# davidfang00/opticalflowdiffusion

Measured on NVIDIA B200. Metric: flows/sec DDIM-50 @436x1024, higher is better.
Workload: dtype bf16

## Files before the change

opticalflowdiffusion_b200/csrc/fd_attention.cu:

```cuda
#include <stdlib.h>

#include "fd_mma.cuh"

using namespace fdmma;

namespace {


constexpr int kLaTile = 64;
constexpr int kLaRowBytes = 2 * kHidden * 2 + 16;
constexpr int kLaTileBytes = kLaTile * kLaRowBytes;
constexpr int kLaSmemBytes = 2 * kLaTileBytes;
constexpr int kLaPartial = 2 * kHidden + kHeads * kD * kD;

__global__ void __launch_bounds__(256, 3) linattn_partial_kernel(const __nv_bfloat16* __restrict__ kv, int row_stride,
                                                              float* __restrict__ partial, int HW, int chunk_px) {
  extern __shared__ __align__(16) uint8_t la_smem[];
  const int n = blockIdx.y, chunk = blockIdx.x;
  const int p_begin = chunk * chunk_px;
  const int p_end = min(HW, p_begin + chunk_px);
  const int t = threadIdx.x, warp = t >> 5, lane = t & 31;
  const int g = lane >> 2, tq = lane & 3;
  const int head = warp & 3, mhalf = warp >> 2;
  const __nv_bfloat16* base = kv + (long)n * HW * row_stride;
// ... 27 lines not shown
      issue_tile(p0 + kLaTile, buf ^ 1);
      cp_async_wait<1>();
    } else {
      cp_async_wait<0>();
    }
    __syncthreads();
    const uint32_t tb = smem0 + buf * kLaTileBytes;
    const int nvalid = p_end - p0;
    uint32_t ka[kLaTile / 16][4];
#pragma unroll
    for (int ks = 0; ks < kLaTile / 16; ++ks)
      ldmatrix_x4_trans(ka[ks], tb + (ks * 16 + (mi >> 1) * 8 + r) * kLaRowBytes + (head * kD + mhalf * 16 + (mi & 1) * 8) * 2);
    float t0 = -INFINITY, t1 = -INFINITY;
#pragma unroll
    for (int ks = 0; ks < kLaTile / 16; ++ks) {
#pragma unroll
      for (int rg = 0; rg < 4; ++rg) {
        const float2 f = fd_unpack_bf16(ka[ks][rg]);
        const int px = ks * 16 + 2 * tq + (rg >> 1) * 8;
        const float a = px < nvalid ? f.x : -INFINITY, b = px + 1 < nvalid ? f.y : -INFINITY;
        if (rg & 1) t1 = fmaxf(t1, fmaxf(a, b)); else t0 = fmaxf(t0, fmaxf(a, b));
      }
    }
    t0 = fmaxf(t0, __shfl_xor_sync(0xffffffffu, t0, 1)); t0 = fmaxf(t0, __shfl_xor_sync(0xffffffffu, t0, 2));
    t1 = fmaxf(t1, __shfl_xor_sync(0xffffffffu, t1, 1)); t1 = fmaxf(t1, __shfl_xor_sync(0xffffffffu, t1, 2));
    const float mn0 = fmaxf(m0, t0), mn1 = fmaxf(m1, t1);
    const float f0 = (m0 == -INFINITY) ? 0.f : __expf(m0 - mn0), f1 = (m1 == -INFINITY) ? 0.f : __expf(m1 - mn1);
    m0 = mn0;
    m1 = mn1;
#pragma unroll
    for (int nt = 0; nt < 4; ++nt) {
      acc[nt][0] *= f0; acc[nt][1] *= f0; acc[nt][2] *= f1; acc[nt][3] *= f1;
    }
    float e0 = 0.f, e1 = 0.f;
#pragma unroll
    for (int ks = 0; ks < kLaTile / 16; ++ks) {
#pragma unroll
      for (int rg = 0; rg < 4; ++rg) {
        const float2 f = fd_unpack_bf16(ka[ks][rg]);
        const int px = ks * 16 + 2 * tq + (rg >> 1) * 8;
        const float mm = (rg & 1) ? mn1 : mn0;
        const float a = px < nvalid ? __expf(f.x - mm) : 0.f, b = px + 1 < nvalid ? __expf(f.y - mm) : 0.f;
        const uint32_t pk = fd_pack_bf16(a, b);
        ka[ks][rg] = pk;
        const float2 rq = fd_unpack_bf16(pk);
        if (rg & 1) e1 += rq.x + rq.y; else e0 += rq.x + rq.y;
      }
    }
    s0 = s0 * f0 + e0;
    s1 = s1 * f1 + e1;
#pragma unroll
    for (int ks = 0; ks < kLaTile / 16; ++ks) {
      uint32_t b01[4], b23[4];
      const uint32_t vb = tb + (ks * 16 + (mi & 1) * 8 + r) * kLaRowBytes + (kHidden + head * kD + (mi >> 1) * 8) * 2;
      ldmatrix_x4_trans(b01, vb);
      ldmatrix_x4_trans(b23, vb + 16 * 2);
      mma_bf16(acc[0], ka[ks], b01[0], b01[1]);
      mma_bf16(acc[1], ka[ks], b01[2], b01[3]);
      mma_bf16(acc[2], ka[ks], b23[0], b23[1]);
      mma_bf16(acc[3], ka[ks], b23[2], b23[3]);
    }
    __syncthreads();
  }
  s0 += __shfl_xor_sync(0xffffffffu, s0, 1); s0 += __shfl_xor_sync(0xffffffffu, s0, 2);
  s1 += __shfl_xor_sync(0xffffffffu, s1, 1); s1 += __shfl_xor_sync(0xffffffffu, s1, 2);
  float* out = partial + ((long)n * gridDim.x + chunk) * kLaPartial;
  if (tq == 0) {
    const int d0 = head * kD + mhalf * 16 + g;
    out[d0] = m0;
    out[d0 + 8] = m1;
    out[kHidden + d0] = s0;
    out[kHidden + d0 + 8] = s1;
  }
  float* c = out + 2 * kHidden + (head * kD + mhalf * 16) * kD;
#pragma unroll
  for (int nt = 0; nt < 4; ++nt) {
    c[g * kD + nt * 8 + 2 * tq] = acc[nt][0];
    c[g * kD + nt * 8 + 2 * tq + 1] = acc[nt][1];
    c[(g + 8) * kD + nt * 8 + 2 * tq] = acc[nt][2];
    c[(g + 8) * kD + nt * 8 + 2 * tq + 1] = acc[nt][3];
  }
}

__global__ void __launch_bounds__(1024) linattn_combine_kernel(const float* __restrict__ partial,
                                                               __nv_bfloat16* __restrict__ ctx_t, int nchunks,
                                                               float inv_hw) {
  const int n = blockIdx.x / kHeads, head = blockIdx.x % kHeads;
  const int d = threadIdx.x >> 5, e = threadIdx.x & 31;
  const float* base = partial + (long)n * nchunks * kLaPartial;
  float M = -INFINITY;
  for (int c = 0; c < nchunks; ++c) M = fmaxf(M, base[(long)c * kLaPartial + head * kD + d]);
  float S = 0.f, acc = 0.f;
  for (int c = 0; c < nchunks; ++c) {
    const float* pc = base + (long)c * kLaPartial;
    const float mc = pc[head * kD + d];
    const float f = (mc == -INFINITY) ? 0.f : __expf(mc - M);
    S += pc[kHidden + head * kD + d] * f;
    acc += pc[2 * kHidden + (head * kD + d) * kD + e] * f;
  }
  ctx_t[((long)n * kHeads + head) * kD * kD + e * kD + d] = __float2bfloat16(acc / S * inv_hw * 0.17677669529663687f);
}

__global__ void __launch_bounds__(1024) linattn_combine_stats_kernel(const float* __restrict__ partial,
                                                                     float* __restrict__ stats, int nchunks, float inv_hw) {
  const int n = blockIdx.x / kHeads, head = blockIdx.x % kHeads;
  const int d = threadIdx.x >> 5, e = threadIdx.x & 31;
  const float* base = partial + (long)n * nchunks * kLaPartial;
  float M = -INFINITY;
  for (int c = 0; c < nchunks; ++c) M = fmaxf(M, base[(long)c * kLaPartial + head * kD + d]);
  float S = 0.f, acc = 0.f;
  for (int c = 0; c < nchunks; ++c) {
    const float* pc = base + (long)c * kLaPartial;
    const float mc = pc[head * kD + d];
    const float f = (mc == -INFINITY) ? 0.f : __expf(mc - M);
    S += pc[kHidden + head * kD + d] * f;
    acc += pc[2 * kHidden + (head * kD + d) * kD + e] * f;
  }
  float* so = stats + (long)n * kLaPartial;
  if (e == 0) {
    so[head * kD + d] = M;
    so[kHidden + head * kD + d] = S;
  }
  so[2 * kHidden + (head * kD + d) * kD + e] = acc / S * inv_hw;
}

constexpr int kApRowBytes = kHidden * 2 + 16;
constexpr int kCtStride = kD + 8;

__global__ void __launch_bounds__(128) linattn_apply_kernel(const __nv_bfloat16* __restrict__ qkv,
                                                            const __nv_bfloat16* __restrict__ ctx_t,
                                                            __nv_bfloat16* __restrict__ out, int HW) {
  __shared__ __align__(16) uint8_t s_q[64 * kApRowBytes];
  __shared__ __align__(16) __nv_bfloat16 s_ct[kHeads * kD * kCtStride];
  const int n = blockIdx.y;
  const int t = threadIdx.x, warp = t >> 5, lane = t & 31;
  const int g = lane >> 2, tq = lane & 3;
  for (int i = t; i < kHeads * kD * kD; i += 128) {
    const int hd = i / kD, d = i % kD;
    s_ct[hd * kCtStride + d] = ctx_t[(long)n * kHeads * kD * kD + i];
  }
  const __nv_bfloat16* base = qkv + (long)n * HW * kQkv;
  const uint32_t sq = smem_addr(s_q);
  const int ntiles = (HW + 63) / 64;
  for (int tile = blockIdx.x; tile < ntiles; tile += gridDim.x) {
    const int p0 = tile * 64;
    __syncthreads();
#pragma unroll
    for (int it = 0; it < (64 * 16) / 128; ++it) {
      const int idx = it * 128 + t;
      const int px = idx >> 4, q16 = idx & 15;
      const bool ok = p0 + px < HW;
      cp_async16(sq + px * kApRowBytes + q16 * 16, base + (long)(ok ? p0 + px : p0) * kQkv + q16 * 8, ok);
    }
    cp_async_commit();
    cp_async_wait<0>();
    __syncthreads();
    const uint32_t wrow = sq + (warp * 16) * kApRowBytes;
    const int mi = lane >> 3, r = lane & 7;
    uint32_t qa[kHeads][2][4];
#pragma unroll
    for (int h = 0; h < kHeads; ++h)
#pragma unroll
      for (int ks = 0; ks < 2; ++ks)
        ldmatrix_x4(qa[h][ks], wrow + ((mi & 1) * 8 + r) * kApRowBytes + (h * kD + ks * 16 + (mi >> 1) * 8) * 2);
    __syncwarp();
#pragma unroll
    for (int h = 0; h < kHeads; ++h) {
      float q0[8], q1[8];
#pragma unroll
      for (int ks = 0; ks < 2; ++ks) {
        const float2 a0 = fd_unpack_bf16(qa[h][ks][0]), a1 = fd_unpack_bf16(qa[h][ks][1]);
        const float2 a2 = fd_unpack_bf16(qa[h][ks][2]), a3 = fd_unpack_bf16(qa[h][ks][3]);
        q0[ks * 4 + 0] = a0.x; q0[ks * 4 + 1] = a0.y; q0[ks * 4 + 2] = a2.x; q0[ks * 4 + 3] = a2.y;
        q1[ks * 4 + 0] = a1.x; q1[ks * 4 + 1] = a1.y; q1[ks * 4 + 2] = a3.x; q1[ks * 4 + 3] = a3.y;
      }
      float m0 = q0[0], m1 = q1[0];
#pragma unroll
      for (int i = 1; i < 8; ++i) { m0 = fmaxf(m0, q0[i]); m1 = fmaxf(m1, q1[i]); }
      m0 = fmaxf(m0, __shfl_xor_sync(0xffffffffu, m0, 1));
      m0 = fmaxf(m0, __shfl_xor_sync(0xffffffffu, m0, 2));
      m1 = fmaxf(m1, __shfl_xor_sync(0xffffffffu, m1, 1));
      m1 = fmaxf(m1, __shfl_xor_sync(0xffffffffu, m1, 2));
      float s0 = 0.f, s1 = 0.f;
#pragma unroll
      for (int i = 0; i < 8; ++i) {
        q0[i] = __expf(q0[i] - m0); s0 += q0[i];
        q1[i] = __expf(q1[i] - m1); s1 += q1[i];
      }
      s0 += __shfl_xor_sync(0xffffffffu, s0, 1);
      s0 += __shfl_xor_sync(0xffffffffu, s0, 2);
      s1 += __shfl_xor_sync(0xffffffffu, s1, 1);
      s1 += __shfl_xor_sync(0xffffffffu, s1, 2);
      const float i0 = __fdividef(1.f, s0), i1 = __fdividef(1.f, s1);
      float o[4][4];
#pragma unroll
      for (int nt = 0; nt < 4; ++nt)
#pragma unroll
        for (int j = 0; j < 4; ++j) o[nt][j] = 0.f;
#pragma unroll
      for (int ks = 0; ks < 2; ++ks) {
// ... 528 lines not shown
```

opticalflowdiffusion_b200/csrc/fd_linattn_tc.cu:

```cuda
#include <stdlib.h>

#include "fd_tc.cuh"

using namespace fdtc;

namespace {

constexpr int kTilePx = 128;
constexpr int kLaEpiWarps = 16;
constexpr int kLaEpi = kLaEpiWarps * 32;
constexpr int kLaThreads = 64 + kLaEpi;
constexpr float kLog2e = 1.4426950408889634f;

__device__ __forceinline__ uint64_t la_desc_mn(uint32_t saddr, uint32_t lbo) {
  uint64_t d = (uint64_t)((saddr & 0x3FFFFu) >> 4);
  d |= (uint64_t)(lbo >> 4) << 16;
  d |= (uint64_t)(1024u >> 4) << 32;
  d |= 1ull << 46;
  d |= 2ull << 61;
  return d;
}
__host__ __device__ constexpr uint32_t la_idesc(int M, int N, bool a_mn, bool b_mn) {
  return (1u << 4) | (1u << 7) | (1u << 10) | ((a_mn ? 1u : 0u) << 15) | ((b_mn ? 1u : 0u) << 16) | ((uint32_t)(N >> 3) << 17) |
         ((uint32_t)(M >> 4) << 24);
// ... 281 lines not shown
      if (!(p.dbg & 4))
        la_row_stats2<C>(x_smem + s * Cf::kXBytes, row, half, 4 + grp * 4 + quarter, s_sx + (u & 1) * 256, p.eps, mu, r, sigma);
      const bool valid = (t0 + i) * kTilePx + row < p.HW;
      const uint64_t nrm2 = pk2(-r * mu, -r * mu), r2 = pk2(r, r);
      const uint64_t rv2 = valid ? r2 : 0ull;
      mbar_wait(pempty(pb), ((i / NP) & 1) ^ 1u);
      mbar_wait(d1full(as), u & 1);
      tc_fence_after();
#pragma unroll
      for (int cc = 0; cc < 2; ++cc) {
        const int col0 = half * 64 + cc * 32;
        uint32_t acc[32];
        tmem_ld32(tmem_base + lane_off + (uint32_t)(as * 128 + col0), acc);
        tmem_ld_wait();
        if (cc == 1) {
          tc_fence_before();
          mbar_arrive(d1empty(as));
        }
        if (p.dbg & 1) continue;
        uint32_t pk[16];
#pragma unroll
        for (int j4 = 0; j4 < 8; ++j4) {
          const ulonglong2 s4 = *reinterpret_cast<const ulonglong2*>(s_sk + col0 + j4 * 4);
          const ulonglong2 m4 = *reinterpret_cast<const ulonglong2*>(s_mk + col0 + j4 * 4);
          const float2 a0 = up2(ffma2(r2, pk2u(acc[j4 * 4 + 0], acc[j4 * 4 + 1]), ffma2(nrm2, s4.x, m4.x)));
          const float2 a1 = up2(ffma2(r2, pk2u(acc[j4 * 4 + 2], acc[j4 * 4 + 3]), ffma2(nrm2, s4.y, m4.y)));
          const float2 p0 = up2(fmul2(pk2(la_ex2(a0.x), la_ex2(a0.y)), rv2));
          const float2 p1 = up2(fmul2(pk2(la_ex2(a1.x), la_ex2(a1.y)), rv2));
          pk[j4 * 2] = fd_pack_bf16(p0.x, p0.y);
          pk[j4 * 2 + 1] = fd_pack_bf16(p1.x, p1.y);
        }
        const uint32_t rbase = p_smem + pb * Cf::kPBytes + half * 16384 + row * 128;
#pragma unroll
        for (int q = 0; q < 4; ++q) {
          const uint32_t piece = (uint32_t)(cc * 4 + q) ^ (uint32_t)(row & 7);
          la_st16(rbase + piece * 16u, pk[q * 4], pk[q * 4 + 1], pk[q * 4 + 2], pk[q * 4 + 3]);
        }
      }
      {
        const float val = half == 0 ? mu : sigma;
        const __nv_bfloat16 hi = __float2bfloat16(val);
        const __nv_bfloat16 lo = __float2bfloat16(val - __bfloat162float(hi));
        const uint32_t abase = aux_smem + pb * Cf::kAuxBytes + (row >> 6) * 2048 + (row & 7) * 2;
        const int g = (row & 63) >> 3;
        const int r0 = half * 2, r1 = half * 2 + 1;
        asm volatile("st.shared.b16 [%0], %1;" ::"r"(abase + r0 * 128 + ((g ^ r0) & 7) * 16), "h"(*reinterpret_cast<const uint16_t*>(&hi))
                     : "memory");
        asm volatile("st.shared.b16 [%0], %1;" ::"r"(abase + r1 * 128 + ((g ^ r1) & 7) * 16), "h"(*reinterpret_cast<const uint16_t*>(&lo))
                     : "memory");
      }
      fence_proxy_async_smem();
      mbar_arrive(pfull(pb));
    }
    mbar_wait(accfull, 0);
    tc_fence_after();
    float* out = p.partial + ((long)blockIdx.x * 128 + row) * (C + 4);
    if (part < C / 32) {
      uint32_t acc[32];
      tmem_ld32(tmem_base + lane_off + (uint32_t)(256 + part * 32), acc);
      tmem_ld_wait();
#pragma unroll
      for (int j4 = 0; j4 < 8; ++j4)
        *reinterpret_cast<float4*>(out + part * 32 + j4 * 4) =
            make_float4(__uint_as_float(acc[j4 * 4]), __uint_as_float(acc[j4 * 4 + 1]), __uint_as_float(acc[j4 * 4 + 2]),
                        __uint_as_float(acc[j4 * 4 + 3]));
    }
    if (part == 3) {
      uint32_t acc[16];
      tmem_ld16(tmem_base + lane_off + 384u, acc);
      tmem_ld_wait();
      *reinterpret_cast<float4*>(out + C) = make_float4(__uint_as_float(acc[0]) + __uint_as_float(acc[1]),
                                                        __uint_as_float(acc[2]) + __uint_as_float(acc[3]), 0.f, 0.f);
    }
  }
  tc_fence_before();
  __syncthreads();
  if (warp == 1) {
    tc_fence_after();
    tmem_dealloc(tmem_base, 512);
  }
}

template <int C>
__global__ void __launch_bounds__(256) linattn_tc_combine_kernel(const float* __restrict__ partial, const float* __restrict__ wv,
                                                                 const float* __restrict__ wout, __nv_bfloat16* __restrict__ mt,
                                                                 int cps, int HW) {
  __shared__ float s_g[32][C + 1];
  __shared__ float s_wv[32][C + 1];
  __shared__ float s_ctx[32][33];
  __shared__ float s_T[32], s_den[32];
  const int n = blockIdx.x, head = blockIdx.y, t = threadIdx.x;
  constexpr int V4 = (C + 4) / 4;
  for (int idx = t; idx < 32 * V4; idx += 256) {
    const int dd = idx / V4, v = idx - dd * V4;
    constexpr int U = 6;
    float4 acc[U];
#pragma unroll
    for (int u = 0; u < U; ++u) acc[u] = make_float4(0.f, 0.f, 0.f, 0.f);
    const float* src = partial + (((long)n * cps) * 128 + head * 32 + dd) * (C + 4) + v * 4;
    constexpr long kStep = 128L * (C + 4);
    int j = 0;
    for (; j + U <= cps; j += U) {
      float4 x[U];
#pragma unroll
      for (int u = 0; u < U; ++u) x[u] = *reinterpret_cast<const float4*>(src + (long)(j + u) * kStep);
#pragma unroll
      for (int u = 0; u < U; ++u) {
        acc[u].x += x[u].x;
        acc[u].y += x[u].y;
        acc[u].z += x[u].z;
        acc[u].w += x[u].w;
      }
    }
    for (int u = 0; j < cps; ++j, ++u) {
      const float4 x = *reinterpret_cast<const float4*>(src + (long)j * kStep);
      acc[u].x += x.x;
      acc[u].y += x.y;
      acc[u].z += x.z;
      acc[u].w += x.w;
    }
    float4 a;
    a.x = ((acc[0].x + acc[1].x) + (acc[2].x + acc[3].x)) + (acc[4].x + acc[5].x);
    a.y = ((acc[0].y + acc[1].y) + (acc[2].y + acc[3].y)) + (acc[4].y + acc[5].y);
    a.z = ((acc[0].z + acc[1].z) + (acc[2].z + acc[3].z)) + (acc[4].z + acc[5].z);
    a.w = ((acc[0].w + acc[1].w) + (acc[2].w + acc[3].w)) + (acc[4].w + acc[5].w);
    if (v < C / 4) {
      s_g[dd][v * 4] = a.x;
      s_g[dd][v * 4 + 1] = a.y;
      s_g[dd][v * 4 + 2] = a.z;
      s_g[dd][v * 4 + 3] = a.w;
    } else {
      s_T[dd] = a.x;
      s_den[dd] = a.y;
    }
  }
  for (int idx = t; idx < 32 * C; idx += 256) {
    const int e = idx / C, c = idx - e * C;
    s_wv[e][c] = __ldg(wv + (long)(head * 32 + e) * C + c);
  }
  __syncthreads();
  for (int o = t; o < 1024; o += 256) {
    const int dd = o >> 5, e = o & 31;
    const float T = s_T[dd];
    float a = 0.f;
#pragma unroll 8
    for (int c = 0; c < C; ++c) a = fmaf(s_g[dd][c] - T, s_wv[e][c], a);
    s_ctx[dd][e] = a * (0.17677669529663687f / (s_den[dd] * (float)HW));
  }
  __syncthreads();
  for (int o = t; o < 32 * C; o += 256) {
    const int dd = o & 31, co = o >> 5;
    const float* w = wout + (long)co * 128 + head * 32;
    float a = 0.f;
#pragma unroll
    for (int e = 0; e < 32; ++e) a = fmaf(s_ctx[dd][e], __ldg(w + e), a);
    mt[((long)n * C + co) * 128 + head * 32 + dd] = __float2bfloat16(a);
  }
}

template <int C>
struct ApTcCfg {
  static constexpr int kChunks = C / 64;
  static constexpr int kXBytes = kChunks * 16384;
  static constexpr int kStages = C == 64 ? 6 : 2;
  static constexpr int kWBytes = kChunks * 16384;
  static constexpr int kMBytes = 2 * C * 128;
  static constexpr int kQBytes = 32768;
  static constexpr int kNQ = C == 64 ? 2 : 1;
  static constexpr int kOBytes = kChunks * 16384;
  static constexpr int kNO = 1;
  static constexpr int kOffW = kStages * kXBytes;
  static constexpr int kOffM = kOffW + kWBytes;
  static constexpr int kOffQ = kOffM + kMBytes;
  static constexpr int kOffO = kOffQ + kNQ * kQBytes;
  static constexpr int kOffConst = kOffO + kNO * kOBytes;
  static constexpr int kOffSx = kOffConst + 2048;
  static constexpr int kOffRs = kOffSx + 8192;
  static constexpr int kOffBar = kOffRs + 2048;
  static constexpr int kSmemBytes = 1024 + kOffBar + 256;
};

struct ApParams {
  int N, HW, cps, tiles;
  float eps;
  const float* sq;
  const float* bout;
  const float* g2;
  int dbg;
};

template <int C>
__global__ void __launch_bounds__(kLaThreads, 1)
linattn_apply_kernel_tc(const __grid_constant__ CUtensorMap map_x, const __grid_constant__ CUtensorMap map_w,
                        const __grid_constant__ CUtensorMap map_m, const __grid_constant__ CUtensorMap map_out, const ApParams p) {
  using Cf = ApTcCfg<C>;
  constexpr int S = Cf::kStages;
  constexpr int NCH = Cf::kChunks;
  constexpr int NQ = Cf::kNQ;
  constexpr int NO = Cf::kNO;
  extern __shared__ uint8_t smem_raw[];
  const uint32_t base = (smem_u32(smem_raw) + 1023u) & ~1023u;
  uint8_t* gbase = smem_raw + (base - smem_u32(smem_raw));
  const uint32_t x_smem = base, w_smem = base + Cf::kOffW, m_smem = base + Cf::kOffM, q_smem = base + Cf::kOffQ,
                 o_smem = base + Cf::kOffO;
  float* s_sq = reinterpret_cast<float*>(gbase + Cf::kOffConst);
  float* s_b = s_sq + 128;
  float* s_g2 = s_b + C;
  float2* s_sx = reinterpret_cast<float2*>(gbase + Cf::kOffSx);
  const uint32_t bar = base + Cf::kOffBar;
  auto xfull = [&](int s) { return bar + 8u * s; };
  auto xempty = [&](int s) { return bar + 8u * (S + s); };
  const uint32_t wfull = bar + 8u * (2 * S);
  auto d1full = [&](int s) { return bar + 8u * (2 * S + 1 + s); };
  auto d1empty = [&](int s) { return bar + 8u * (2 * S + 3 + s); };
  auto qfull = [&](int s) { return bar + 8u * (2 * S + 5 + s); };
  auto qempty = [&](int s) { return bar + 8u * (2 * S + 7 + s); };
  auto d2full = [&](int s) { return bar + 8u * (2 * S + 9 + s); };
  auto d2empty = [&](int s) { return bar + 8u * (2 * S + 11 + s); };
  auto sfull = [&](int s) { return bar + 8u * (2 * S + 13 + s); };
  uint32_t* s_tmem = reinterpret_cast<uint32_t*>(gbase + Cf::kOffBar + 8 * (2 * S + 15));

  const int warp = threadIdx.x >> 5, lane = threadIdx.x & 31;
  const int n = blockIdx.x / p.cps, jc = blockIdx.x % p.cps;
  const int t0 = (int)((long)jc * p.tiles / p.cps), t1 = (int)((long)(jc + 1) * p.tiles / p.cps);
  const int nt = t1 - t0;

  if (warp == 0 && lane == 0) {
    tma_prefetch_desc(&map_x);
    tma_prefetch_desc(&map_w);
    tma_prefetch_desc(&map_m);
    tma_prefetch_desc(&map_out);
    for (int s = 0; s < S; ++s) {
      mbar_init(xfull(s), 1);
      mbar_init(xempty(s), kLaEpi / 2);
    }
    mbar_init(wfull, 1);
    for (int s = 0; s < 2; ++s) {
      mbar_init(sfull(s), kLaEpi / 2);
      mbar_init(d1full(s), 1);
      mbar_init(d1empty(s), kLaEpi / 2);
      mbar_init(qfull(s), kLaEpi / 2);
      mbar_init(qempty(s), 1);
      mbar_init(d2full(s), 1);
      mbar_init(d2empty(s), kLaEpi / 2);
    }
    fence_barrier_init();
  }
  if (warp == 1) tmem_alloc(smem_u32(s_tmem), 512);
  tc_fence_before();
  __syncthreads();
  tc_fence_after();
  const uint32_t tmem_base = *s_tmem;
  fd_grid_dependency_wait();

  if (warp == 0) {
    if (elect_one_sync()) {
      mbar_expect_tx(wfull, Cf::kWBytes + Cf::kMBytes);
      for (int ch = 0; ch < NCH; ++ch) tma_load_2d(w_smem + ch * 16384, &map_w, wfull, ch * 64, 0);
      for (int dc = 0; dc < 2; ++dc) tma_load_3d(m_smem + dc * (C * 128), &map_m, wfull, dc * 64, 0, n);
      for (int i = 0; i < nt; ++i) {
        const int s = i % S;
        mbar_wait(xempty(s), ((i / S) & 1) ^ 1u);
        mbar_expect_tx(xfull(s), Cf::kXBytes);
        for (int ch = 0; ch < NCH; ++ch)
          tma_load_3d(x_smem + s * Cf::kXBytes + ch * 16384, &map_x, xfull(s), ch * 64, (t0 + i) * kTilePx, n);
      }
    }
  } else if (warp == 1) {
    if (elect_one_sync()) {
      constexpr uint32_t id1 = la_idesc(128, 128, false, false);
      constexpr uint32_t id2 = la_idesc(128, C, false, false);
      mbar_wait(wfull, 0);
      const uint64_t wdesc = umma_desc_sw128(w_smem), mdesc = umma_desc_sw128(m_smem);
      auto mma1 = [&](int i) {
        const int as = i & 1, s = i % S;
        mbar_wait(d1empty(as), ((i >> 1) & 1) ^ 1u);
        mbar_wait(xfull(s), (i / S) & 1);
        tc_fence_after();
        const uint64_t xd = umma_desc_sw128(x_smem + s * Cf::kXBytes);
        if (!(p.dbg & 8)) {
#pragma unroll
          for (int ch = 0; ch < NCH; ++ch)
#pragma unroll
            for (int k = 0; k < 4; ++k)
              umma_bf16(tmem_base + as * 128, xd + (uint64_t)(ch * 1024 + 2 * k), wdesc + (uint64_t)(ch * 1024 + 2 * k), id1,
                        (ch | k) != 0 ? 1u : 0u);
        }
        umma_commit(d1full(as));
      };
      if (nt > 0) mma1(0);
      for (int i = 0; i < nt; ++i) {
        if (i + 1 < nt) mma1(i + 1);
        const int qb = i % NQ, as = i & 1;
        mbar_wait(qfull(qb), (i / NQ) & 1);
        mbar_wait(d2empty(as), ((i >> 1) & 1) ^ 1u);
        tc_fence_after();
        const uint64_t qd = umma_desc_sw128(q_smem + qb * Cf::kQBytes);
        if (!(p.dbg & 2)) {
#pragma unroll
          for (int ks = 0; ks < 8; ++ks)
            umma_bf16(tmem_base + 256 + as * 128, qd + (uint64_t)((ks >> 2) * 1024 + 2 * (ks & 3)),
                      mdesc + (uint64_t)((ks >> 2) * (C * 128 >> 4) + 2 * (ks & 3)), id2, ks != 0 ? 1u : 0u);
        }
        umma_commit(d2full(as));
        umma_commit(qempty(qb));
      }
    }
    __syncwarp();
  } else {
    const int ew = warp - 2, et = threadIdx.x - 64;
    const int grp = ew >> 3, half = (ew >> 2) & 1, quarter = warp & 3;
    const int row = quarter * 32 + lane;
    for (int i = et; i < 128 + 2 * C; i += kLaEpi)
      s_sq[i] = i < 128 ? __ldg(p.sq + i) : (i < 128 + C ? __ldg(p.bout + i - 128) : __ldg(p.g2 + i - 128 - C));
    named_bar_sync(1, kLaEpi);
    const uint32_t lane_off = (uint32_t)(quarter * 32) << 16;

    float2* s_rs = reinterpret_cast<float2*>(gbase + Cf::kOffRs);
    if (grp == 0) {
      for (int i = 0; i < nt; ++i) {
        const int qb = i % NQ, as = i & 1;
        mbar_wait(sfull(i & 1), (i >> 1) & 1);
        const float2 st = s_rs[(i & 1) * 128 + row];
        const float r = st.y;
        const uint64_t nrm2 = pk2(-r * st.x, -r * st.x), r2 = pk2(r, r);
        mbar_wait(qempty(qb), ((i / NQ) & 1) ^ 1u);
        mbar_wait(d1full(as), (i >> 1) & 1);
        tc_fence_after();
        uint32_t acc[2][32];
        tmem_ld32(tmem_base + lane_off + (uint32_t)(as * 128 + half * 64), acc[0]);
        tmem_ld32(tmem_base + lane_off + (uint32_t)(as * 128 + half * 64 + 32), acc[1]);
        tmem_ld_wait();
        tc_fence_before();
        mbar_arrive(d1empty(as));
        if (p.dbg & 1) {
          fence_proxy_async_smem();
          mbar_arrive(qfull(qb));
          continue;
        }
        float mx[2] = {-INFINITY, -INFINITY};
#pragma unroll
        for (int hh = 0; hh < 2; ++hh) {
          const int col0 = (half * 2 + hh) * 32;
#pragma unroll
          for (int j4 = 0; j4 < 8; ++j4) {
            const ulonglong2 s4 = *reinterpret_cast<const ulonglong2*>(s_sq + col0 + j4 * 4);
            const float2 a0 = up2(ffma2(r2, pk2u(acc[hh][j4 * 4 + 0], acc[hh][j4 * 4 + 1]), fmul2(nrm2, s4.x)));
            const float2 a1 = up2(ffma2(r2, pk2u(acc[hh][j4 * 4 + 2], acc[hh][j4 * 4 + 3]), fmul2(nrm2, s4.y)));
            acc[hh][j4 * 4 + 0] = __float_as_uint(a0.x);
            acc[hh][j4 * 4 + 1] = __float_as_uint(a0.y);
            acc[hh][j4 * 4 + 2] = __float_as_uint(a1.x);
            acc[hh][j4 * 4 + 3] = __float_as_uint(a1.y);
            mx[hh] = fmaxf(mx[hh], fmaxf(fmaxf(a0.x, a0.y), fmaxf(a1.x, a1.y)));
          }
        }
        float sum[2] = {0.f, 0.f};
#pragma unroll
        for (int j = 0; j < 32; ++j) {
#pragma unroll
          for (int hh = 0; hh < 2; ++hh) {
            const float e = la_ex2(__uint_as_float(acc[hh][j]) - mx[hh]);
            acc[hh][j] = __float_as_uint(e);
            sum[hh] += e;
          }
        }
        const uint32_t rbase = q_smem + qb * Cf::kQBytes + half * 16384 + row * 128;
#pragma unroll
        for (int hh = 0; hh < 2; ++hh) {
          const float inv = __fdividef(1.f, sum[hh]);
          const uint64_t inv2 = pk2(inv, inv);
#pragma unroll
          for (int q = 0; q < 4; ++q) {
            uint32_t w[4];
#pragma unroll
            for (int e = 0; e < 4; ++e) {
              const float2 f = up2(fmul2(pk2u(acc[hh][q * 8 + e * 2], acc[hh][q * 8 + e * 2 + 1]), inv2));
              w[e] = fd_pack_bf16(f.x, f.y);
            }
            const uint32_t piece = (uint32_t)(hh * 4 + q) ^ (uint32_t)(row & 7);
            la_st16(rbase + piece * 16u, w[0], w[1], w[2], w[3]);
          }
        }
        fence_proxy_async_smem();
        mbar_arrive(qfull(qb));
      }
    } else {
      constexpr int CPT = C / 2;
      const int gw = ew - 8;
      const int col0 = half * CPT;
      uint32_t slab_count = 0;
      auto x_stats = [&](int j) {
        const int sj = j % S;
        mbar_wait(xfull(sj), (j / S) & 1);
        float mu = 0.f, r = 1.f, sigma = 1.f;
        if (!(p.dbg & 4)) la_row_stats2<C>(x_smem + sj * Cf::kXBytes, row, half, 8 + quarter, s_sx + (j & 1) * 256, p.eps, mu, r, sigma);
        if (half == 0) s_rs[(j & 1) * 128 + row] = make_float2(mu, r);
        mbar_arrive(sfull(j & 1));
      };
// ... 14 lines not shown
          for (int j = 0; j < 16; ++j) {
            const uint64_t x = fadd2(pk2u(acc[2 * j], acc[2 * j + 1]), *reinterpret_cast<const uint64_t*>(s_b + col0 + cb * 32 + 2 * j));
            o[cb * 16 + j] = x;
            sm2 = fadd2(sm2, x);
            sq22 = ffma2(x, x, sq22);
          }
        }
        tc_fence_before();
        mbar_arrive(d2empty(as));
        const uint32_t ob = slab_count % NO;
        ++slab_count;
        if (p.dbg & 16) {
          mbar_arrive(xempty(s));
          continue;
        }
        const float2 smf = up2(sm2), sqf = up2(sq22);
        const float sm = smf.x + smf.y, sq2 = sqf.x + sqf.y;
        float2* sx = s_sx + 512 + (i & 1) * 256;
        sx[half * 128 + row] = make_float2(sm, sq2);
        if (gw == 0 && elect_one_sync()) tma_store_wait_read<NO - 1>();
        named_bar_sync(2, kLaEpi / 2);
        const float2 other = sx[(half ^ 1) * 128 + row];
        const float mean = (sm + other.x) * (1.f / C);
        const float var = fmaxf((sq2 + other.y) * (1.f / C) - mean * mean, 0.f);
        const float rstd = rsqrtf(var + p.eps);
        const uint64_t rstd2 = pk2(rstd, rstd), nmr2 = pk2(-mean * rstd, -mean * rstd);
#pragma unroll
        for (int cb = 0; cb < CPT / 32; ++cb) {
          const int c0 = col0 + cb * 32;
          const int chunk = c0 >> 6, g0 = (c0 & 63) >> 3;
          const uint32_t xrow = x_smem + s * Cf::kXBytes + chunk * 16384 + row * 128;
          const uint32_t orow = o_smem + ob * Cf::kOBytes + chunk * 16384 + row * 128;
#pragma unroll
          for (int q = 0; q < 4; ++q) {
            const uint32_t piece = (uint32_t)(g0 + q) ^ (uint32_t)(row & 7);
            const uint4 xr = la_ld16(xrow + piece * 16u);
            const uint32_t xw[4] = {xr.x, xr.y, xr.z, xr.w};
            uint32_t ow[4];
#pragma unroll
            for (int e = 0; e < 4; ++e) {
              const float2 f = fd_unpack_bf16(xw[e]);
              const uint64_t nrm = ffma2(o[cb * 16 + q * 4 + e], rstd2, nmr2);
              const float2 y = up2(ffma2(nrm, *reinterpret_cast<const uint64_t*>(s_g2 + c0 + q * 8 + e * 2), pk2(f.x, f.y)));
              ow[e] = fd_pack_bf16(y.x, y.y);
            }
            la_st16(orow + piece * 16u, ow[0], ow[1], ow[2], ow[3]);
          }
        }
        fence_proxy_async_smem();
        mbar_arrive(xempty(s));
        named_bar_sync(3, kLaEpi / 2);
        if (gw == 0 && elect_one_sync() && !(p.dbg & 32)) {
          for (int ch = 0; ch < NCH; ++ch)
            la_tma_store_3d(&map_out, o_smem + ob * Cf::kOBytes + ch * 16384, ch * 64, (t0 + i) * kTilePx, n);
          tma_store_commit();
        }
      }
      __syncwarp();
      if (gw == 0 && elect_one_sync()) tma_store_wait_all();
    }
  }
  tc_fence_before();
  __syncthreads();
  if (warp == 1) {
    tc_fence_after();
    tmem_dealloc(tmem_base, 512);
  }
}

int ctas_per_sample(int N, int tiles) {
  int cps = FD_NUM_SMS / N;
  if (cps < 1) cps = 1;
  if (cps > tiles) cps = tiles;
  return cps;
}

template <int C>
int run_tc(const void* x, const void* wk, const float* sk, const float* mk, const void* wq, const float* sq, const float* wv,
           const float* wout, const float* bout, const float* g2, void* out, float* workspace, int N, int HW, float eps,
           cudaStream_t st) {
  const int tiles = (HW + kTilePx - 1) / kTilePx;
  const int cps = ctas_per_sample(N, tiles);
  float* partial = workspace;
  __nv_bfloat16* mt = reinterpret_cast<__nv_bfloat16*>(workspace + (size_t)N * cps * 128 * (C + 4));
  CUtensorMap map_x, map_wk, map_wq, map_m, map_out;
  {
    const uint64_t dims[3] = {(uint64_t)C, (uint64_t)HW, (uint64_t)N};
    const uint64_t str[2] = {(uint64_t)C * 2, (uint64_t)HW * C * 2};
    const uint32_t box[3] = {64, (uint32_t)kTilePx, 1};
    if (int e = make_tmap_bf16(&map_x, x, 3, dims, str, box)) return e;
    if (int e = make_tmap_bf16(&map_out, out, 3, dims, str, box)) return e;
  }
  {
    const uint64_t dims[2] = {(uint64_t)C, 128};
    const uint64_t str[1] = {(uint64_t)C * 2};
    const uint32_t box[2] = {64, 128};
    if (int e = make_tmap_bf16(&map_wk, wk, 2, dims, str, box)) return e;
    if (int e = make_tmap_bf16(&map_wq, wq, 2, dims, str, box)) return e;
  }
  {
    const uint64_t dims[3] = {128, (uint64_t)C, (uint64_t)N};
    const uint64_t str[2] = {256, (uint64_t)C * 256};
    const uint32_t box[3] = {64, (uint32_t)C, 1};
    if (int e = make_tmap_bf16(&map_m, mt, 3, dims, str, box)) return e;
  }
  static bool attr_set = false;
  if (!attr_set) {
    FD_CUDA(cudaFuncSetAttribute(linattn_ctx_kernel<C>, cudaFuncAttributeMaxDynamicSharedMemorySize, CtxCfg<C>::kSmemBytes));
    FD_CUDA(cudaFuncSetAttribute(linattn_apply_kernel_tc<C>, cudaFuncAttributeMaxDynamicSharedMemorySize, ApTcCfg<C>::kSmemBytes));
    attr_set = true;
  }
  static int la_dbg = -1;
  if (la_dbg < 0) { const char* e = getenv("FD_LA_DBG"); la_dbg = e ? atoi(e) : 0; }
  CtxParams cp{N, HW, cps, tiles, eps, sk, mk, partial, la_dbg & 15};
  FD_CUDA(fd_launch_pdl(linattn_ctx_kernel<C>, dim3(N * cps), dim3(kLaThreads), CtxCfg<C>::kSmemBytes, st, map_x, map_wk, cp));
  FD_LAUNCH_CHECK();
  linattn_tc_combine_kernel<C><<<dim3(N, 4), 256, 0, st>>>(partial, wv, wout, mt, cps, HW);
  FD_LAUNCH_CHECK();
  ApParams ap{N, HW, cps, tiles, eps, sq, bout, g2, la_dbg >> 4};
  FD_CUDA(fd_launch_pdl(linattn_apply_kernel_tc<C>, dim3(N * cps), dim3(kLaThreads), ApTcCfg<C>::kSmemBytes, st, map_x, map_wq, map_m,
                        map_out, ap));
  FD_LAUNCH_CHECK();
  return FD_OK;
}

}

extern "C" {

size_t fd_linattn_tc_workspace_floats(int N, int HW, int C) {
  const int tiles = (HW + kTilePx - 1) / kTilePx;
  const int cps = ctas_per_sample(N > 0 ? N : 1, tiles > 0 ? tiles : 1);
  return (size_t)N * cps * 128 * (C + 4) + (size_t)N * C * 128 / 2 + 64;
}

int fd_linattn_tc_prep(const float* wqkv, const float* g1, void* wq, float* sq, void* wk, float* sk, float* mk, float* wv, int C,
                       void* stream) {
  FD_REQUIRE(wqkv && g1 && wq && sq && wk && sk && mk && wv, "linattn_tc_prep: null pointer");
  FD_REQUIRE(C == 64 || C == 128, "linattn_tc_prep: C=%d not in {64,128}", C);
  linattn_tc_prep_kernel<<<384, 128, 0, (cudaStream_t)stream>>>(wqkv, g1, static_cast<__nv_bfloat16*>(wq), sq,
                                                               static_cast<__nv_bfloat16*>(wk), sk, mk, wv, C);
  FD_LAUNCH_CHECK();
  return FD_OK;
}

int fd_linattn_tc(const void* x, const void* wk, const float* sk, const float* mk, const void* wq, const float* sq,
                  const float* wv, const float* wout, const float* bout, const float* g2, void* out, float* workspace, int N,
                  int HW, int C, float eps, void* stream) {
  FD_REQUIRE(x && wk && sk && mk && wq && sq && wv && wout && bout && g2 && out && workspace, "linattn_tc: null pointer");
  FD_REQUIRE(N > 0 && HW > 0, "linattn_tc: bad geometry N=%d HW=%d", N, HW);
  FD_REQUIRE(C == 64 || C == 128, "linattn_tc: C=%d not in {64,128}", C);
  cudaStream_t st = (cudaStream_t)stream;
  if (C == 64) return run_tc<64>(x, wk, sk, mk, wq, sq, wv, wout, bout, g2, out, workspace, N, HW, eps, st);
  return run_tc<128>(x, wk, sk, mk, wq, sq, wv, wout, bout, g2, out, workspace, N, HW, eps, st);
}

}
```

Baseline: 9.451.

## Fuse linear-attention combine into apply kernel and unroll chunk combine loops

Removes the separate combine kernel launch in the tensor-core linear attention path. Each apply CTA's epilogue warps now reduce the per-chunk partials, form ctx and the fused Wout matrix, and write it swizzled into shared memory, signalling the MMA warp through an mbarrier. This drops a launch and the global round-trip for the M matrix, but every CTA of a sample redundantly repeats the reduction over all chunks. It also batches loads by eight in the older mma-path combine kernels to expose memory-level parallelism.

```diff
diff --git a/opticalflowdiffusion_b200/csrc/fd_attention.cu b/opticalflowdiffusion_b200/csrc/fd_attention.cu
--- a/opticalflowdiffusion_b200/csrc/fd_attention.cu
+++ b/opticalflowdiffusion_b200/csrc/fd_attention.cu
@@ -133,22 +133,55 @@
   }
 }
 
+__device__ __forceinline__ void la_combine_chunks(const float* __restrict__ base, int nchunks, int head, int d, int e, float& M,
+                                                  float& S, float& acc) {
+  constexpr int kB = 8;
+  const float* pm = base + head * kD + d;
+  const float* ps = base + kHidden + head * kD + d;
+  const float* pa = base + 2 * kHidden + (head * kD + d) * kD + e;
+  M = -INFINITY;
+  int c = 0;
+  for (; c + kB <= nchunks; c += kB) {
+    float m[kB];
+#pragma unroll
+    for (int u = 0; u < kB; ++u) m[u] = pm[(long)(c + u) * kLaPartial];
+#pragma unroll
+    for (int u = 0; u < kB; ++u) M = fmaxf(M, m[u]);
+  }
+  for (; c < nchunks; ++c) M = fmaxf(M, pm[(long)c * kLaPartial]);
+  S = 0.f;
+  acc = 0.f;
+  auto fold = [&](float mc, float sc, float ac) {
+    const float f = (mc == -INFINITY) ? 0.f : __expf(mc - M);
+    S += sc * f;
+    acc += ac * f;
+  };
+  c = 0;
+  for (; c + kB <= nchunks; c += kB) {
+    float m[kB], sv[kB], a[kB];
+#pragma unroll
+    for (int u = 0; u < kB; ++u) {
+      const long o = (long)(c + u) * kLaPartial;
+      m[u] = pm[o];
+      sv[u] = ps[o];
+      a[u] = pa[o];
+    }
+#pragma unroll
+    for (int u = 0; u < kB; ++u) fold(m[u], sv[u], a[u]);
+  }
+  for (; c < nchunks; ++c) {
+    const long o = (long)c * kLaPartial;
+    fold(pm[o], ps[o], pa[o]);
+  }
+}
+
 __global__ void __launch_bounds__(1024) linattn_combine_kernel(const float* __restrict__ partial,
                                                                __nv_bfloat16* __restrict__ ctx_t, int nchunks,
                                                                float inv_hw) {
   const int n = blockIdx.x / kHeads, head = blockIdx.x % kHeads;
   const int d = threadIdx.x >> 5, e = threadIdx.x & 31;
-  const float* base = partial + (long)n * nchunks * kLaPartial;
-  float M = -INFINITY;
-  for (int c = 0; c < nchunks; ++c) M = fmaxf(M, base[(long)c * kLaPartial + head * kD + d]);
-  float S = 0.f, acc = 0.f;
-  for (int c = 0; c < nchunks; ++c) {
-    const float* pc = base + (long)c * kLaPartial;
-    const float mc = pc[head * kD + d];
-    const float f = (mc == -INFINITY) ? 0.f : __expf(mc - M);
-    S += pc[kHidden + head * kD + d] * f;
-    acc += pc[2 * kHidden + (head * kD + d) * kD + e] * f;
-  }
+  float M, S, acc;
+  la_combine_chunks(partial + (long)n * nchunks * kLaPartial, nchunks, head, d, e, M, S, acc);
   ctx_t[((long)n * kHeads + head) * kD * kD + e * kD + d] = __float2bfloat16(acc / S * inv_hw * 0.17677669529663687f);
 }
 
@@ -156,17 +189,8 @@
                                                                      float* __restrict__ stats, int nchunks, float inv_hw) {
   const int n = blockIdx.x / kHeads, head = blockIdx.x % kHeads;
   const int d = threadIdx.x >> 5, e = threadIdx.x & 31;
-  const float* base = partial + (long)n * nchunks * kLaPartial;
-  float M = -INFINITY;
-  for (int c = 0; c < nchunks; ++c) M = fmaxf(M, base[(long)c * kLaPartial + head * kD + d]);
-  float S = 0.f, acc = 0.f;
-  for (int c = 0; c < nchunks; ++c) {
-    const float* pc = base + (long)c * kLaPartial;
-    const float mc = pc[head * kD + d];
-    const float f = (mc == -INFINITY) ? 0.f : __expf(mc - M);
-    S += pc[kHidden + head * kD + d] * f;
-    acc += pc[2 * kHidden + (head * kD + d) * kD + e] * f;
-  }
+  float M, S, acc;
+  la_combine_chunks(partial + (long)n * nchunks * kLaPartial, nchunks, head, d, e, M, S, acc);
   float* so = stats + (long)n * kLaPartial;
   if (e == 0) {
     so[head * kD + d] = M;
diff --git a/opticalflowdiffusion_b200/csrc/fd_linattn_tc.cu b/opticalflowdiffusion_b200/csrc/fd_linattn_tc.cu
--- a/opticalflowdiffusion_b200/csrc/fd_linattn_tc.cu
+++ b/opticalflowdiffusion_b200/csrc/fd_linattn_tc.cu
@@ -387,80 +387,111 @@
 }
 
 template <int C>
-__global__ void __launch_bounds__(256) linattn_tc_combine_kernel(const float* __restrict__ partial, const float* __restrict__ wv,
-                                                                 const float* __restrict__ wout, __nv_bfloat16* __restrict__ mt,
-                                                                 int cps, int HW) {
-  __shared__ float s_g[32][C + 1];
-  __shared__ float s_wv[32][C + 1];
-  __shared__ float s_ctx[32][33];
-  __shared__ float s_T[32], s_den[32];
-  const int n = blockIdx.x, head = blockIdx.y, t = threadIdx.x;
+__device__ __forceinline__ void la_combine_to_smem(const float* __restrict__ partial, const float* __restrict__ wv,
+                                                   const float* __restrict__ wout, int n, int cps, int HW, uint32_t m_smem,
+                                                   float* scratch, int et) {
+  constexpr int P = C + 4;
+  float(*s_g)[P] = reinterpret_cast<float(*)[P]>(scratch);
+  float(*s_wv)[P] = reinterpret_cast<float(*)[P]>(scratch + 32 * P);
+  float(*s_ctx)[33] = reinterpret_cast<float(*)[33]>(scratch + 64 * P);
+  float* s_T = scratch + 64 * P + 32 * 33;
+  float* s_den = s_T + 32;
   constexpr int V4 = (C + 4) / 4;
-  for (int idx = t; idx < 32 * V4; idx += 256) {
-    const int dd = idx / V4, v = idx - dd * V4;
-    constexpr int U = 6;
-    float4 acc[U];
-#pragma unroll
-    for (int u = 0; u < U; ++u) acc[u] = make_float4(0.f, 0.f, 0.f, 0.f);
-    const float* src = partial + (((long)n * cps) * 128 + head * 32 + dd) * (C + 4) + v * 4;
-    constexpr long kStep = 128L * (C + 4);
-    int j = 0;
-    for (; j + U <= cps; j += U) {
-      float4 x[U];
-#pragma unroll
-      for (int u = 0; u < U; ++u) x[u] = *reinterpret_cast<const float4*>(src + (long)(j + u) * kStep);
-#pragma unroll
-      for (int u = 0; u < U; ++u) {
-        acc[u].x += x[u].x;
-        acc[u].y += x[u].y;
-        acc[u].z += x[u].z;
-        acc[u].w += x[u].w;
-      }
-    }
-    for (int u = 0; j < cps; ++j, ++u) {
-      const float4 x = *reinterpret_cast<const float4*>(src + (long)j * kStep);
-      acc[u].x += x.x;
-      acc[u].y += x.y;
-      acc[u].z += x.z;
-      acc[u].w += x.w;
-    }
-    float4 a;
-    a.x = ((acc[0].x + acc[1].x) + (acc[2].x + acc[3].x)) + (acc[4].x + acc[5].x);
-    a.y = ((acc[0].y + acc[1].y) + (acc[2].y + acc[3].y)) + (acc[4].y + acc[5].y);
-    a.z = ((acc[0].z + acc[1].z) + (acc[2].z + acc[3].z)) + (acc[4].z + acc[5].z);
-    a.w = ((acc[0].w + acc[1].w) + (acc[2].w + acc[3].w)) + (acc[4].w + acc[5].w);
-    if (v < C / 4) {
-      s_g[dd][v * 4] = a.x;
-      s_g[dd][v * 4 + 1] = a.y;
-      s_g[dd][v * 4 + 2] = a.z;
-      s_g[dd][v * 4 + 3] = a.w;
-    } else {
-      s_T[dd] = a.x;
-      s_den[dd] = a.y;
-    }
-  }
-  for (int idx = t; idx < 32 * C; idx += 256) {
-    const int e = idx / C, c = idx - e * C;
-    s_wv[e][c] = __ldg(wv + (long)(head * 32 + e) * C + c);
-  }
-  __syncthreads();
-  for (int o = t; o < 1024; o += 256) {
-    const int dd = o >> 5, e = o & 31;
-    const float T = s_T[dd];
-    float a = 0.f;
-#pragma unroll 8
-    for (int c = 0; c < C; ++c) a = fmaf(s_g[dd][c] - T, s_wv[e][c], a);
-    s_ctx[dd][e] = a * (0.17677669529663687f / (s_den[dd] * (float)HW));
-  }
-  __syncthreads();
-  for (int o = t; o < 32 * C; o += 256) {
-    const int dd = o & 31, co = o >> 5;
-    const float* w = wout + (long)co * 128 + head * 32;
-    float a = 0.f;
-#pragma unroll
-    for (int e = 0; e < 32; ++e) a = fmaf(s_ctx[dd][e], __ldg(w + e), a);
-    mt[((long)n * C + co) * 128 + head * 32 + dd] = __float2bfloat16(a);
-  }
+  constexpr int U = 6;
+  constexpr long kStep = 128L * (C + 4);
+  const int lane = et & 31, w = et >> 5;
+  for (int head = 0; head < 4; ++head) {
+    for (int idx = et; idx < 32 * V4; idx += kLaEpi) {
+      const int dd = idx / V4, v = idx - dd * V4;
+      float4 acc[U];
+#pragma unroll
+      for (int u = 0; u < U; ++u) acc[u] = make_float4(0.f, 0.f, 0.f, 0.f);
+      const float* src = partial + (((long)n * cps) * 128 + head * 32 + dd) * (C + 4) + v * 4;
+      int j = 0;
+      for (; j + U <= cps; j += U) {
+        float4 x[U];
+#pragma unroll
+        for (int u = 0; u < U; ++u) x[u] = *reinterpret_cast<const float4*>(src + (long)(j + u) * kStep);
+#pragma unroll
+        for (int u = 0; u < U; ++u) {
+          acc[u].x += x[u].x;
+          acc[u].y += x[u].y;
+          acc[u].z += x[u].z;
+          acc[u].w += x[u].w;
+        }
+      }
+#pragma unroll
+      for (int u = 0; u < U - 1; ++u) {
+        if (j + u < cps) {
+          const float4 x = *reinterpret_cast<const float4*>(src + (long)(j + u) * kStep);
+          acc[u].x += x.x;
+          acc[u].y += x.y;
+          acc[u].z += x.z;
+          acc[u].w += x.w;
+        }
+      }
+      float4 a;
+      a.x = ((acc[0].x + acc[1].x) + (acc[2].x + acc[3].x)) + (acc[4].x + acc[5].x);
+      a.y = ((acc[0].y + acc[1].y) + (acc[2].y + acc[3].y)) + (acc[4].y + acc[5].y);
+      a.z = ((acc[0].z + acc[1].z) + (acc[2].z + acc[3].z)) + (acc[4].z + acc[5].z);
+      a.w = ((acc[0].w + acc[1].w) + (acc[2].w + acc[3].w)) + (acc[4].w + acc[5].w);
+      if (v < C / 4) {
+        *reinterpret_cast<float4*>(&s_g[dd][v * 4]) = a;
+      } else {
+        s_T[dd] = a.x;
+        s_den[dd] = a.y;
+      }
+    }
+    for (int idx = et; idx < 32 * (C / 4); idx += kLaEpi) {
+      const int e = idx / (C / 4), c4 = idx - e * (C / 4);
+      *reinterpret_cast<float4*>(&s_wv[e][c4 * 4]) = __ldg(reinterpret_cast<const float4*>(wv + (long)(head * 32 + e) * C) + c4);
+    }
+    named_bar_sync(1, kLaEpi);
+    {
+      const int e = lane, d0 = w, d1 = w + 16;
+      const float T0 = s_T[d0], T1 = s_T[d1];
+      float a0 = 0.f, a1 = 0.f;
+#pragma unroll 4
+      for (int c = 0; c < C; c += 4) {
+        const float4 g0 = *reinterpret_cast<const float4*>(&s_g[d0][c]);
+        const float4 g1 = *reinterpret_cast<const float4*>(&s_g[d1][c]);
+        const float4 wv4 = *reinterpret_cast<const float4*>(&s_wv[e][c]);
+        a0 = fmaf(g0.x - T0, wv4.x, a0);
+        a1 = fmaf(g1.x - T1, wv4.x, a1);
+        a0 = fmaf(g0.y - T0, wv4.y, a0);
+        a1 = fmaf(g1.y - T1, wv4.y, a1);
+        a0 = fmaf(g0.z - T0, wv4.z, a0);
+        a1 = fmaf(g1.z - T1, wv4.z, a1);
+        a0 = fmaf(g0.w - T0, wv4.w, a0);
+        a1 = fmaf(g1.w - T1, wv4.w, a1);
+      }
+      s_ctx[d0][e] = a0 * (0.17677669529663687f / (s_den[d0] * (float)HW));
+      s_ctx[d1][e] = a1 * (0.17677669529663687f / (s_den[d1] * (float)HW));
+    }
+    named_bar_sync(1, kLaEpi);
+    {
+      const int dd = lane, d = head * 32 + dd;
+      const uint32_t dst = m_smem + (uint32_t)(d >> 6) * (C * 128) + (uint32_t)(d & 7) * 2;
+      const uint32_t g = (uint32_t)((d & 63) >> 3);
+      for (int co = w; co < C; co += kLaEpiWarps) {
+        const float4* wr = reinterpret_cast<const float4*>(wout + (long)co * 128 + head * 32);
+        float a = 0.f;
+#pragma unroll
+        for (int e4 = 0; e4 < 8; ++e4) {
+          const float4 w4 = __ldg(wr + e4);
+          a = fmaf(s_ctx[dd][e4 * 4 + 0], w4.x, a);
+          a = fmaf(s_ctx[dd][e4 * 4 + 1], w4.y, a);
+          a = fmaf(s_ctx[dd][e4 * 4 + 2], w4.z, a);
+          a = fmaf(s_ctx[dd][e4 * 4 + 3], w4.w, a);
+        }
+        const __nv_bfloat16 b = __float2bfloat16(a);
+        asm volatile("st.shared.b16 [%0], %1;" ::"r"(dst + (uint32_t)co * 128 + ((g ^ (uint32_t)(co & 7)) << 4)),
+                     "h"(*reinterpret_cast<const uint16_t*>(&b))
+                     : "memory");
+      }
+    }
+  }
+  named_bar_sync(1, kLaEpi);
 }
 
 template <int C>
@@ -483,11 +514,15 @@
   static constexpr int kOffRs = kOffSx + 8192;
   static constexpr int kOffBar = kOffRs + 2048;
   static constexpr int kSmemBytes = 1024 + kOffBar + 256;
+  static_assert((kOffConst - kOffQ) / 4 >= 64 * (C + 4) + 32 * 33 + 64, "combine scratch");
 };
 
 struct ApParams {
   int N, HW, cps, tiles;
   float eps;
+  const float* partial;
+  const float* wv;
+  const float* wout;
   const float* sq;
   const float* bout;
   const float* g2;
@@ -497,7 +532,7 @@
 template <int C>
 __global__ void __launch_bounds__(kLaThreads, 1)
 linattn_apply_kernel_tc(const __grid_constant__ CUtensorMap map_x, const __grid_constant__ CUtensorMap map_w,
-                        const __grid_constant__ CUtensorMap map_m, const __grid_constant__ CUtensorMap map_out, const ApParams p) {
+                        const __grid_constant__ CUtensorMap map_out, const ApParams p) {
   using Cf = ApTcCfg<C>;
   constexpr int S = Cf::kStages;
   constexpr int NCH = Cf::kChunks;
@@ -523,7 +558,8 @@
   auto d2full = [&](int s) { return bar + 8u * (2 * S + 9 + s); };
   auto d2empty = [&](int s) { return bar + 8u * (2 * S + 11 + s); };
   auto sfull = [&](int s) { return bar + 8u * (2 * S + 13 + s); };
-  uint32_t* s_tmem = reinterpret_cast<uint32_t*>(gbase + Cf::kOffBar + 8 * (2 * S + 15));
+  const uint32_t mfull = bar + 8u * (2 * S + 15);
+  uint32_t* s_tmem = reinterpret_cast<uint32_t*>(gbase + Cf::kOffBar + 8 * (2 * S + 16));
 
   const int warp = threadIdx.x >> 5, lane = threadIdx.x & 31;
   const int n = blockIdx.x / p.cps, jc = blockIdx.x % p.cps;
@@ -533,7 +569,6 @@
   if (warp == 0 && lane == 0) {
     tma_prefetch_desc(&map_x);
     tma_prefetch_desc(&map_w);
-    tma_prefetch_desc(&map_m);
     tma_prefetch_desc(&map_out);
     for (int s = 0; s < S; ++s) {
       mbar_init(xfull(s), 1);
@@ -549,6 +584,7 @@
       mbar_init(d2full(s), 1);
       mbar_init(d2empty(s), kLaEpi / 2);
     }
+    mbar_init(mfull, kLaEpi);
     fence_barrier_init();
   }
   if (warp == 1) tmem_alloc(smem_u32(s_tmem), 512);
@@ -560,9 +596,8 @@
 
   if (warp == 0) {
     if (elect_one_sync()) {
-      mbar_expect_tx(wfull, Cf::kWBytes + Cf::kMBytes);
+      mbar_expect_tx(wfull, Cf::kWBytes);
       for (int ch = 0; ch < NCH; ++ch) tma_load_2d(w_smem + ch * 16384, &map_w, wfull, ch * 64, 0);
-      for (int dc = 0; dc < 2; ++dc) tma_load_3d(m_smem + dc * (C * 128), &map_m, wfull, dc * 64, 0, n);
       for (int i = 0; i < nt; ++i) {
         const int s = i % S;
         mbar_wait(xempty(s), ((i / S) & 1) ^ 1u);
@@ -594,6 +629,7 @@
         umma_commit(d1full(as));
       };
       if (nt > 0) mma1(0);
+      mbar_wait(mfull, 0);
       for (int i = 0; i < nt; ++i) {
         if (i + 1 < nt) mma1(i + 1);
         const int qb = i % NQ, as = i & 1;
@@ -618,7 +654,9 @@
     const int row = quarter * 32 + lane;
     for (int i = et; i < 128 + 2 * C; i += kLaEpi)
       s_sq[i] = i < 128 ? __ldg(p.sq + i) : (i < 128 + C ? __ldg(p.bout + i - 128) : __ldg(p.g2 + i - 128 - C));
-    named_bar_sync(1, kLaEpi);
+    la_combine_to_smem<C>(p.partial, p.wv, p.wout, n, p.cps, p.HW, m_smem, reinterpret_cast<float*>(gbase + Cf::kOffQ), et);
+    fence_proxy_async_smem();
+    mbar_arrive(mfull);
     const uint32_t lane_off = (uint32_t)(quarter * 32) << 16;
 
     float2* s_rs = reinterpret_cast<float2*>(gbase + Cf::kOffRs);
@@ -799,8 +837,7 @@
   const int tiles = (HW + kTilePx - 1) / kTilePx;
   const int cps = ctas_per_sample(N, tiles);
   float* partial = workspace;
-  __nv_bfloat16* mt = reinterpret_cast<__nv_bfloat16*>(workspace + (size_t)N * cps * 128 * (C + 4));
-  CUtensorMap map_x, map_wk, map_wq, map_m, map_out;
+  CUtensorMap map_x, map_wk, map_wq, map_out;
   {
     const uint64_t dims[3] = {(uint64_t)C, (uint64_t)HW, (uint64_t)N};
     const uint64_t str[2] = {(uint64_t)C * 2, (uint64_t)HW * C * 2};
@@ -815,12 +852,6 @@
     if (int e = make_tmap_bf16(&map_wk, wk, 2, dims, str, box)) return e;
     if (int e = make_tmap_bf16(&map_wq, wq, 2, dims, str, box)) return e;
   }
-  {
-    const uint64_t dims[3] = {128, (uint64_t)C, (uint64_t)N};
-    const uint64_t str[2] = {256, (uint64_t)C * 256};
-    const uint32_t box[3] = {64, (uint32_t)C, 1};
-    if (int e = make_tmap_bf16(&map_m, mt, 3, dims, str, box)) return e;
-  }
   static bool attr_set = false;
   if (!attr_set) {
     FD_CUDA(cudaFuncSetAttribute(linattn_ctx_kernel<C>, cudaFuncAttributeMaxDynamicSharedMemorySize, CtxCfg<C>::kSmemBytes));
@@ -832,10 +863,8 @@
   CtxParams cp{N, HW, cps, tiles, eps, sk, mk, partial, la_dbg & 15};
   FD_CUDA(fd_launch_pdl(linattn_ctx_kernel<C>, dim3(N * cps), dim3(kLaThreads), CtxCfg<C>::kSmemBytes, st, map_x, map_wk, cp));
   FD_LAUNCH_CHECK();
-  linattn_tc_combine_kernel<C><<<dim3(N, 4), 256, 0, st>>>(partial, wv, wout, mt, cps, HW);
-  FD_LAUNCH_CHECK();
-  ApParams ap{N, HW, cps, tiles, eps, sq, bout, g2, la_dbg >> 4};
-  FD_CUDA(fd_launch_pdl(linattn_apply_kernel_tc<C>, dim3(N * cps), dim3(kLaThreads), ApTcCfg<C>::kSmemBytes, st, map_x, map_wq, map_m,
+  ApParams ap{N, HW, cps, tiles, eps, partial, wv, wout, sq, bout, g2, la_dbg >> 4};
+  FD_CUDA(fd_launch_pdl(linattn_apply_kernel_tc<C>, dim3(N * cps), dim3(kLaThreads), ApTcCfg<C>::kSmemBytes, st, map_x, map_wq,
                         map_out, ap));
   FD_LAUNCH_CHECK();
   return FD_OK;
@@ -848,7 +877,7 @@
 size_t fd_linattn_tc_workspace_floats(int N, int HW, int C) {
   const int tiles = (HW + kTilePx - 1) / kTilePx;
   const int cps = ctas_per_sample(N > 0 ? N : 1, tiles > 0 ? tiles : 1);
-  return (size_t)N * cps * 128 * (C + 4) + (size_t)N * C * 128 / 2 + 64;
+  return (size_t)N * cps * 128 * (C + 4);
 }
 
 int fd_linattn_tc_prep(const float* wqkv, const float* g1, void* wq, float* sq, void* wk, float* sk, float* mk, float* wv, int C,
```

New measurement: 9.410, median of 6. About the same (-0.4%).
